# AdmiralenOla/Scoary

Hardware: AMD Instinct MI355X
Metric: gene x permutation Fisher tests/sec (higher is better)
Workload: dtype u32 bit-words (bit-sliced adders / AND + popcount), f64 for Fisher p; 1 GPU; cfg3: 50000 genes x 2000 isolates x 10 traits, --permute 10000 per GPU; counts + Fisher + label permutations + exceedance counts; gene_kind=config, gene_order=config, gene_partition=every rank its own genes (weak scaling), genes_per_gpu=50000, genes_total=50000, isolates=2000, traits=10, permutations=10000, parallelism=gene-shard x1, hip_graph=False, hip_graph_auto=False, label_tiles=generated on every rank, exchange=none (single GPU)

## Files before the change

include/scoary_hip.h:

```cpp
#ifndef SCOARY_HIP_H
#define SCOARY_HIP_H

#include <stdint.h>

#ifdef __cplusplus
extern "C" {
#endif

#define SCOARY_ABI_VERSION 11

#define SCOARY_OK 0
#define SCOARY_ERR_ARG (-1)
#define SCOARY_ERR_HIP (-2)
#define SCOARY_ERR_SIZE (-3)
#define SCOARY_ERR_DEVICE (-4)

typedef struct scoary_ctx *scoary_handle;
typedef void *scoary_stream_t;

int scoary_abi_version(void);

int scoary_create(int device, scoary_handle *out);
void scoary_destroy(scoary_handle h);
const char *scoary_last_error(scoary_handle h);
// ... 1 lines not shown
int64_t scoary_tiled_quads(int64_t N);
int64_t scoary_tiled_genes(int64_t G);
int64_t scoary_tiled_bytes(int64_t G, int64_t N);
int64_t scoary_row_words(int64_t N);

int scoary_pack_dense(scoary_handle h, const uint8_t *d_dense, int64_t G,
                      int64_t N, uint32_t *d_tiled, scoary_stream_t stream);
int scoary_tile_rows(scoary_handle h, const uint64_t *d_rows64, int64_t G,
                     int64_t N, uint32_t *d_tiled, scoary_stream_t stream);

int scoary_counts(scoary_handle h, const uint32_t *d_tiled,
                  const uint32_t *d_traits, const uint32_t *d_masks, int64_t G,
                  int64_t T, int64_t N, int32_t *d_counts, int32_t *d_margins,
                  scoary_stream_t stream);
int64_t scoary_counts_traits_per_pass(int64_t T);
int64_t scoary_trait_plan_bytes(int64_t T, int64_t N);
int scoary_trait_plan(scoary_handle h, const uint32_t *d_traits, const uint32_t *d_masks,
                      int64_t T, int64_t N, int32_t *d_margins, int32_t *d_mask_class,
                      void *d_plan, scoary_stream_t stream);
int scoary_counts_planned(scoary_handle h, const uint32_t *d_tiled, const void *d_plan,
                          const int32_t *d_margins, int64_t G, int64_t T, int64_t N,
                          int32_t *d_counts, scoary_stream_t stream);

int scoary_fisher(scoary_handle h, const int32_t *d_tables, int64_t M,
                  double *d_p, double *d_or, uint32_t *d_crit,
                  scoary_stream_t stream);
int64_t scoary_fisher_scipy_max_isolates(void);
int scoary_fisher_scipy(scoary_handle h, const int32_t *d_tables, int64_t M, double *d_p,
                        uint64_t *d_skipped, scoary_stream_t stream);
int scoary_fisher_lists(scoary_handle h, const int32_t *d_tables, int64_t T, int64_t G,
                        const int32_t *d_lorder, const uint8_t *d_lflipped,
                        double *d_p, double *d_or, uint32_t *d_crit, uint32_t *d_lcrit,
                        scoary_stream_t stream);

int64_t scoary_perm_max_isolates(void);
int scoary_perm_generate(scoary_handle h, const uint32_t *d_masks,
                         const int32_t *d_margins, int64_t T, int64_t N,
                         int64_t P, int64_t perm_base, int64_t trait_base,
                         uint64_t seed, uint32_t *d_perms, scoary_stream_t stream);

int scoary_permute(scoary_handle h, const uint32_t *d_tiled,
                   const uint32_t *d_perms, const uint32_t *d_crit, int64_t G,
                   int64_t T, int64_t N, int64_t P, uint32_t *d_r,
                   scoary_stream_t stream);

int scoary_permute_seq(scoary_handle h, const uint32_t *d_tiled, const uint32_t *d_perms,
                       const uint32_t *d_crit, const uint32_t *d_thr, int64_t G, int64_t T,
                       int64_t N, int64_t P, int64_t perm_base, uint32_t *d_r,
                       uint32_t *d_nstop, scoary_stream_t stream);

int64_t scoary_minp_fill_scratch_bytes(int64_t entries);
int scoary_minp_plan(scoary_handle h, const int32_t *d_counts, int64_t T, int64_t G, int64_t *d_off,
                     int32_t *d_lo, int64_t *entries_out, scoary_stream_t stream);
int scoary_minp_fill(scoary_handle h, const int32_t *d_counts, const int64_t *d_off,
                     const int32_t *d_lo, int64_t T, int64_t G, int64_t entries, void *d_scratch,
                     double *d_tab, scoary_stream_t stream);
int scoary_permute_minp(scoary_handle h, const uint32_t *d_tiled, const uint32_t *d_perms,
                        const int64_t *d_off, const int32_t *d_lo, const double *d_tab, int64_t G,
                        int64_t T, int64_t N, int64_t P, int64_t perm_base, int64_t minp_stride,
                        double *d_minp, scoary_stream_t stream);

int64_t scoary_stepdown_chunks(scoary_handle h, int64_t G, int64_t T, int64_t P);
int64_t scoary_stepdown_scratch_bytes(scoary_handle h, int64_t G, int64_t T, int64_t N, int64_t P);
int scoary_permute_stepdown(scoary_handle h, const uint32_t *d_tiled, const uint32_t *d_perms,
                            const int64_t *d_off, const int32_t *d_lo, const double *d_tab,
                            const int32_t *d_order, const double *d_psorted, int64_t G, int64_t T,
                            int64_t N, int64_t P, int64_t perm_base, int64_t minp_stride,
                            double *d_minp, uint32_t *d_c, void *d_scratch, scoary_stream_t stream);

int64_t scoary_list_tiles_words(int64_t N, int64_t P, int64_t T);
int64_t scoary_list_tile_words(int64_t N);
int64_t scoary_list_max_isolates(void);
int64_t scoary_list_segments(int64_t N);
int scoary_list_params(int64_t N, int64_t *out5);
int scoary_perm_generate_tiles(scoary_handle h, const uint32_t *d_masks,
                               const int32_t *d_margins, int64_t T, int64_t N, int64_t P,
                               int64_t perm_base, int64_t trait_base, uint64_t seed,
                               uint32_t *d_tiles, scoary_stream_t stream);
int scoary_perm_generate_tiles_range(scoary_handle h, const uint32_t *d_masks,
                                     const int32_t *d_margins, int64_t T, int64_t N, int64_t P,
                                     int64_t perm_base, int64_t trait_base, uint64_t seed,
                                     int64_t first_tile, int64_t n_tiles, uint32_t *d_tiles,
                                     scoary_stream_t stream);
int scoary_perm_max_strata(void);
int64_t scoary_perm_strata_max_isolates(void);
int scoary_strata_margins(scoary_handle h, const uint32_t *d_labels, const uint32_t *d_masks,
                          const uint16_t *d_strata, int64_t T, int64_t N, int64_t S,
                          int32_t *d_smargins, scoary_stream_t stream);
int scoary_perm_generate_strata(scoary_handle h, const uint32_t *d_masks, const uint16_t *d_strata,
                                const int32_t *d_members, const int32_t *d_offsets,
                                const int32_t *d_smargins, int64_t T, int64_t N, int64_t S, int64_t P,
                                int64_t perm_base, int64_t trait_base, uint64_t seed,
                                uint32_t *d_perms, scoary_stream_t stream);
int scoary_perm_generate_tiles_strata_range(scoary_handle h, const uint32_t *d_masks,
                                            const uint16_t *d_strata, const int32_t *d_members,
                                            const int32_t *d_offsets, const int32_t *d_smargins,
                                            int64_t T, int64_t N, int64_t S, int64_t P,
                                            int64_t perm_base, int64_t trait_base, uint64_t seed,
                                            int64_t first_tile, int64_t n_tiles, uint32_t *d_tiles,
                                            scoary_stream_t stream);
int64_t scoary_cmh_scratch_bytes(int64_t N);
int scoary_cmh(scoary_handle h, const uint32_t *d_tiled, const uint32_t *d_labels, const uint32_t *d_masks,
               const uint16_t *d_strata, const int32_t *d_members, const int32_t *d_offsets,
               const int32_t *d_smargins, int64_t G, int64_t T, int64_t N, int64_t S, double *d_stat,
               double *d_p, double *d_odds, double *d_e2, double *d_var, int32_t *d_a, uint32_t *d_crit,
               int32_t *d_scounts, void *d_scratch, scoary_stream_t stream);
int scoary_cmh_minp_plan(scoary_handle h, const uint32_t *d_tiled, const uint32_t *d_masks,
                         const uint16_t *d_strata, const int32_t *d_members, const int32_t *d_offsets,
                         const int32_t *d_smargins, int64_t G, int64_t T, int64_t N, int64_t S,
                         void *d_scratch, int64_t *d_off, int32_t *d_lo, int64_t *entries_out,
                         scoary_stream_t stream);
int scoary_cmh_minp_fill(scoary_handle h, const double *d_e2, const double *d_var, const int64_t *d_off,
                         const int32_t *d_lo, int64_t T, int64_t G, int64_t entries, double *d_tab,
                         scoary_stream_t stream);
int64_t scoary_cmh_exact_max_isolates(void);
int scoary_cmh_exact(scoary_handle h, const uint32_t *d_tiled, const uint32_t *d_masks, const uint16_t *d_strata,
                     const int32_t *d_members, const int32_t *d_offsets, const int32_t *d_smargins, int64_t G,
                     int64_t T, int64_t N, int64_t S, const int32_t *d_a, const uint32_t *d_crit,
                     const int64_t *d_off, const int32_t *d_lo, int64_t entries, double *d_p, double *d_p_region,
                     double *d_tab, void *d_scratch, scoary_stream_t stream);
int scoary_cmh_exact_odds(scoary_handle h, const uint32_t *d_tiled, const uint32_t *d_masks,
                          const uint16_t *d_strata, const int32_t *d_members, const int32_t *d_offsets,
                          const int32_t *d_smargins, int64_t G, int64_t T, int64_t N, int64_t S,
                          const int32_t *d_a, const int64_t *d_off, const int32_t *d_lo, int64_t entries, double half,
                          double *d_or, double *d_or_lo, double *d_or_hi, void *d_scratch,
                          scoary_stream_t stream);
int scoary_cmh_homogeneity(scoary_handle h, const uint32_t *d_tiled, const uint32_t *d_labels,
                           const uint32_t *d_masks, const uint16_t *d_strata, const int32_t *d_members,
                           const int32_t *d_offsets, const int32_t *d_smargins, int64_t G, int64_t T, int64_t N,
                           int64_t S, const double *d_odds, double *d_stat_bd, double *d_stat_tarone, int32_t *d_df,
                           double *d_p, void *d_scratch, scoary_stream_t stream);
int64_t scoary_permute_lists_scratch_bytes(int64_t G, int64_t T, int64_t N, int64_t P);
int scoary_permute_lists(scoary_handle h, const uint32_t *d_tiles, const uint32_t *d_lidx,
                         int64_t entries, const int32_t *d_lstart, const int32_t *d_lngroups,
                         const int32_t *d_lorder, const uint8_t *d_lflipped,
                         const uint32_t *d_crit, const uint32_t *d_lcrit,
                         const int32_t *d_margins, void *d_scratch,
                         int64_t G, int64_t T, int64_t N, int64_t P, uint32_t *d_r,
                         int accumulate, scoary_stream_t stream);

#define SCOARY_MFMA_ROUTE_NONE 0
#define SCOARY_MFMA_ROUTE_ALL 1
#define SCOARY_MFMA_ROUTE_AUTO 2
int64_t scoary_mfma_max_isolates(void);
int64_t scoary_mfma_panels_bytes(int64_t G, int64_t N);
int64_t scoary_mfma_bfrag_bytes(int64_t N, int64_t P, int64_t T);
int64_t scoary_mfma_breakeven_entries(void);
int scoary_mfma_panels_build(scoary_handle h, const uint32_t *d_tiled, int64_t G, int64_t N,
                             const int32_t *d_order, const uint8_t *d_flipped, void *d_panels,
                             scoary_stream_t stream);
int scoary_set_mfma_route(scoary_handle h, int mode);
int64_t scoary_mfma_route(scoary_handle h, const int64_t *block_start, int64_t G, int64_t T,
                          int64_t N, int64_t P);
int scoary_permute_hybrid(scoary_handle h, const uint32_t *d_tiles, const uint32_t *d_lidx,
                          int64_t entries, const int32_t *d_lstart, const int32_t *d_lngroups,
                          const int32_t *d_lorder, const uint8_t *d_lflipped,
                          const uint32_t *d_crit, const uint32_t *d_lcrit,
                          const int32_t *d_margins, void *d_scratch,
                          int64_t G, int64_t T, int64_t N, int64_t P, uint32_t *d_r,
                          int accumulate, const void *d_panels, void *d_bfrag, int64_t k_split,
                          int64_t routed_entries, scoary_stream_t stream);

int64_t scoary_lists_scratch_bytes(int64_t G, int64_t N);
int64_t scoary_lists_slack_entries(void);
int scoary_lists_plan(scoary_handle h, const uint32_t *d_tiled, int64_t G, int64_t N,
                      void *d_scratch, int32_t *d_start, int32_t *d_ngroups, int32_t *d_order,
                      uint8_t *d_flipped, int64_t *entries_out, scoary_stream_t stream);
int scoary_lists_fill(scoary_handle h, const uint32_t *d_tiled, int64_t G, int64_t N,
                      const void *d_scratch, const int32_t *d_order, const uint8_t *d_flipped,
                      int64_t entries, uint32_t *d_idx, scoary_stream_t stream);


int scoary_hamming(scoary_handle h, const uint32_t *d_tiled, const uint32_t *d_vecrows,
                   int64_t R, int64_t N, int32_t *d_out, scoary_stream_t stream);

int64_t scoary_upgma_scratch_bytes(int64_t n);
int scoary_upgma(scoary_handle h, const int32_t *d_counts, int64_t n, int64_t ncols, void *d_scratch,
                 int32_t *d_merges, int32_t *d_status, scoary_stream_t stream);

int scoary_gather_bits(scoary_handle h, const uint32_t *d_rows, int64_t R, int64_t Wsrc,
                       const int32_t *d_index, int64_t K, uint32_t *d_out,
                       scoary_stream_t stream);

int scoary_tree_pairs(scoary_handle h, const int32_t *d_ops, int64_t nops, int64_t stack_depth,
                      const uint32_t *d_gene_bits, const uint32_t *d_label_bits, int64_t G,
                      int64_t L, int64_t K, int32_t *d_out, scoary_stream_t stream);

int scoary_tree_permute(scoary_handle h, const int32_t *d_ops, int64_t nops,
                        int64_t stack_depth, const uint32_t *d_gene_bits,
                        const uint32_t *d_label_bits, int64_t G, int64_t L, int64_t K,
                        const int32_t *d_obs, uint8_t *d_exceed, scoary_stream_t stream);

int scoary_row_hash(scoary_handle h, const uint32_t *d_tiled, const uint32_t *d_masks,
                    int64_t G, int64_t T, int64_t N, uint64_t *d_out, scoary_stream_t stream);

int scoary_pack_records(scoary_handle h, const int32_t *d_counts, const double *d_p,
                        const double *d_odds, const uint32_t *d_r, const uint32_t *d_nstop,
                        int64_t M, uint32_t *d_rec, scoary_stream_t stream);

int scoary_gather(scoary_handle h, void *rccl_dl, void *comm, const void *d_send, void *d_recv,
                  int64_t bytes, int rank, int nranks, int root, scoary_stream_t stream);

typedef struct scoary_graph *scoary_graph_t;
int scoary_graph_begin(scoary_handle h, scoary_stream_t stream);
int scoary_graph_end(scoary_handle h, scoary_stream_t stream, scoary_graph_t *out);
int scoary_graph_launch(scoary_handle h, scoary_graph_t g, scoary_stream_t stream);
void scoary_graph_destroy(scoary_graph_t g);

int scoary_set_timing(scoary_handle h, int enabled);
int scoary_last_kernel_ms(scoary_handle h, const char *kernel, double *ms_out);

#ifdef __cplusplus
}
#endif
#endif
```

scoary_amd/_abi.py:

```python
import ctypes
import os

_HERE = os.path.dirname(os.path.abspath(__file__))
LIB_PATH = os.environ.get("SCOARY_HIP_LIB") or os.path.join(_HERE, "csrc", "libscoary_hip.so")
HEADER_PATH = os.path.join(os.path.dirname(_HERE), "include", "scoary_hip.h")

ABI_VERSION = 11
PERM_MAX_STRATA = 1024
PERM_STRATA_MAX_ISOLATES = 20479

_i64, _u64, _i32, _vp, _cp = (ctypes.c_int64, ctypes.c_uint64, ctypes.c_int,
                              ctypes.c_void_p, ctypes.c_char_p)

SIGNATURES = {
    "scoary_abi_version": (_i32, []),
    "scoary_create": (_i32, [_i32, ctypes.POINTER(_vp)]),
    "scoary_destroy": (None, [_vp]),
    "scoary_last_error": (_cp, [_vp]),
    "scoary_tiled_quads": (_i64, [_i64]),
    "scoary_tiled_genes": (_i64, [_i64]),
    "scoary_tiled_bytes": (_i64, [_i64, _i64]),
    "scoary_row_words": (_i64, [_i64]),
    "scoary_pack_dense": (_i32, [_vp, _vp, _i64, _i64, _vp, _vp]),
    "scoary_tile_rows": (_i32, [_vp, _vp, _i64, _i64, _vp, _vp]),
    "scoary_counts": (_i32, [_vp, _vp, _vp, _vp, _i64, _i64, _i64, _vp, _vp, _vp]),
    "scoary_counts_traits_per_pass": (_i64, [_i64]),
    "scoary_trait_plan_bytes": (_i64, [_i64, _i64]),
    "scoary_trait_plan": (_i32, [_vp, _vp, _vp, _i64, _i64, _vp, _vp, _vp, _vp]),
    "scoary_counts_planned": (_i32, [_vp, _vp, _vp, _vp, _i64, _i64, _i64, _vp, _vp]),
    "scoary_fisher": (_i32, [_vp, _vp, _i64, _vp, _vp, _vp, _vp]),
    "scoary_fisher_lists": (_i32, [_vp, _vp, _i64, _i64] + [_vp] * 7),
    "scoary_fisher_scipy": (_i32, [_vp, _vp, _i64, _vp, _vp, _vp]),
    "scoary_fisher_scipy_max_isolates": (_i64, []),
    "scoary_perm_generate": (_i32, [_vp, _vp, _vp, _i64, _i64, _i64, _i64, _i64, _u64, _vp, _vp]),
    "scoary_permute": (_i32, [_vp, _vp, _vp, _vp, _i64, _i64, _i64, _i64, _vp, _vp]),
    "scoary_permute_seq": (_i32, [_vp, _vp, _vp, _vp, _vp, _i64, _i64, _i64, _i64, _i64, _vp, _vp,
                                  _vp]),
    "scoary_minp_fill_scratch_bytes": (_i64, [_i64]),
    "scoary_minp_plan": (_i32, [_vp, _vp, _i64, _i64, _vp, _vp, ctypes.POINTER(_i64), _vp]),
    "scoary_minp_fill": (_i32, [_vp, _vp, _vp, _vp, _i64, _i64, _i64, _vp, _vp, _vp]),
    "scoary_permute_minp": (_i32, [_vp] * 6 + [_i64] * 6 + [_vp, _vp]),
    "scoary_stepdown_chunks": (_i64, [_vp, _i64, _i64, _i64]),
    "scoary_stepdown_scratch_bytes": (_i64, [_vp, _i64, _i64, _i64, _i64]),
    "scoary_permute_stepdown": (_i32, [_vp] * 8 + [_i64] * 6 + [_vp] * 4),
    "scoary_list_tiles_words": (_i64, [_i64, _i64, _i64]),
    "scoary_list_tile_words": (_i64, [_i64]),
    "scoary_list_params": (_i32, [_i64, _vp]),
    "scoary_list_max_isolates": (_i64, []),
    "scoary_list_segments": (_i64, [_i64]),
    "scoary_perm_generate_tiles": (_i32, [_vp, _vp, _vp, _i64, _i64, _i64, _i64, _i64, _u64, _vp,
                                          _vp]),
    "scoary_perm_generate_tiles_range": (_i32, [_vp, _vp, _vp, _i64, _i64, _i64, _i64, _i64, _u64, _i64,
                                                _i64, _vp, _vp]),
    "scoary_perm_max_isolates": (_i64, []),
    "scoary_perm_max_strata": (_i32, []),
    "scoary_perm_strata_max_isolates": (_i64, []),
    "scoary_strata_margins": (_i32, [_vp, _vp, _vp, _vp, _i64, _i64, _i64, _vp, _vp]),
    "scoary_perm_generate_strata": (_i32, [_vp] * 6 + [_i64] * 6 + [_u64, _vp, _vp]),
    "scoary_perm_generate_tiles_strata_range": (_i32, [_vp] * 6 + [_i64] * 6 + [_u64, _i64, _i64, _vp, _vp]),
    "scoary_cmh_scratch_bytes": (_i64, [_i64]),
    "scoary_cmh": (_i32, [_vp] * 8 + [_i64] * 4 + [_vp] * 10),
    "scoary_cmh_minp_plan": (_i32, [_vp] * 7 + [_i64] * 4 + [_vp] * 3 + [ctypes.POINTER(_i64), _vp]),
    "scoary_cmh_minp_fill": (_i32, [_vp] * 5 + [_i64] * 3 + [_vp, _vp]),
    "scoary_cmh_exact_max_isolates": (_i64, []),
    "scoary_cmh_exact": (_i32, [_vp] * 7 + [_i64] * 4 + [_vp] * 4 + [_i64] + [_vp] * 5),
    "scoary_cmh_exact_odds": (_i32, [_vp] * 7 + [_i64] * 4 + [_vp] * 3 + [_i64, ctypes.c_double] + [_vp] * 5),
    "scoary_cmh_homogeneity": (_i32, [_vp] * 8 + [_i64] * 4 + [_vp] * 7),
    "scoary_permute_lists_scratch_bytes": (_i64, [_i64, _i64, _i64, _i64]),
    "scoary_permute_lists": (_i32, [_vp, _vp, _vp, _i64] + [_vp] * 8 + [_i64, _i64, _i64, _i64, _vp,
                                                                       _i32, _vp]),
    "scoary_mfma_max_isolates": (_i64, []),
    "scoary_mfma_panels_bytes": (_i64, [_i64, _i64]),
    "scoary_mfma_bfrag_bytes": (_i64, [_i64, _i64, _i64]),
    "scoary_mfma_breakeven_entries": (_i64, []),
    "scoary_mfma_panels_build": (_i32, [_vp, _vp, _i64, _i64, _vp, _vp, _vp, _vp]),
    "scoary_set_mfma_route": (_i32, [_vp, _i32]),
    "scoary_mfma_route": (_i64, [_vp, _vp, _i64, _i64, _i64, _i64]),
    "scoary_permute_hybrid": (_i32, [_vp, _vp, _vp, _i64] + [_vp] * 8 + [_i64, _i64, _i64, _i64, _vp,
                                                                        _i32, _vp, _vp, _i64, _i64, _vp]),
    "scoary_lists_scratch_bytes": (_i64, [_i64, _i64]),
    "scoary_lists_slack_entries": (_i64, []),
    "scoary_lists_plan": (_i32, [_vp, _vp, _i64, _i64, _vp, _vp, _vp, _vp, _vp,
                                 ctypes.POINTER(_i64), _vp]),
    "scoary_lists_fill": (_i32, [_vp, _vp, _i64, _i64, _vp, _vp, _vp, _i64, _vp, _vp]),
    "scoary_hamming": (_i32, [_vp, _vp, _vp, _i64, _i64, _vp, _vp]),
    "scoary_upgma_scratch_bytes": (_i64, [_i64]),
    "scoary_upgma": (_i32, [_vp, _vp, _i64, _i64, _vp, _vp, _vp, _vp]),
    "scoary_gather_bits": (_i32, [_vp, _vp, _i64, _i64, _vp, _i64, _vp, _vp]),
    "scoary_tree_pairs": (_i32, [_vp, _vp, _i64, _i64, _vp, _vp, _i64, _i64, _i64, _vp, _vp]),
    "scoary_tree_permute": (_i32, [_vp, _vp, _i64, _i64, _vp, _vp, _i64, _i64, _i64, _vp, _vp,
                                   _vp]),
    "scoary_row_hash": (_i32, [_vp, _vp, _vp, _i64, _i64, _i64, _vp, _vp]),
    "scoary_pack_records": (_i32, [_vp, _vp, _vp, _vp, _vp, _vp, _i64, _vp, _vp]),
    "scoary_gather": (_i32, [_vp, _vp, _vp, _vp, _vp, _i64, _i32, _i32, _i32, _vp]),
    "scoary_graph_begin": (_i32, [_vp, _vp]),
    "scoary_graph_end": (_i32, [_vp, _vp, ctypes.POINTER(_vp)]),
    "scoary_graph_launch": (_i32, [_vp, _vp, _vp]),
    "scoary_graph_destroy": (None, [_vp]),
    "scoary_set_timing": (_i32, [_vp, _i32]),
    "scoary_last_kernel_ms": (_i32, [_vp, _cp, ctypes.POINTER(ctypes.c_double)]),
}

_lib = None


class ScoaryHipError(RuntimeError):
    pass


def load():
    global _lib
    if _lib is not None:
        return _lib
    if not os.path.exists(LIB_PATH):
        raise ScoaryHipError(
            "HIP extension not built: %s is missing. Run "
            "`python -c 'import __graft_entry__ as g; g.build()'` (needs hipcc). "
            "scoary_amd has no CPU fallback." % LIB_PATH)
    try:
        import torch
    except ImportError:
        pass
    lib = ctypes.CDLL(LIB_PATH, mode=ctypes.RTLD_GLOBAL)
    for name, (res, args) in SIGNATURES.items():
        fn = getattr(lib, name)
        fn.restype = res
        fn.argtypes = args
    got = lib.scoary_abi_version()
    if got != ABI_VERSION:
        raise ScoaryHipError("ABI version mismatch: library %d, binding %d" % (got, ABI_VERSION))
    if (lib.scoary_perm_max_strata(), lib.scoary_perm_strata_max_isolates()) != \
            (PERM_MAX_STRATA, PERM_STRATA_MAX_ISOLATES):
        raise ScoaryHipError("the library's strata limits differ from the binding's")
    _lib = lib
    return lib
```

scoary_amd/csrc/scoary_common.hpp:

```cpp
#ifndef SCOARY_COMMON_HPP
#define SCOARY_COMMON_HPP
#include <hip/hip_runtime.h>

#include <algorithm>
#include <cmath>
#include <cstdint>
#include <cstdio>
#include <cstdlib>
#include <cstring>
#include <string>
#include <utility>
#include <vector>

#include "scoary_hip.h"

struct scoary_ctx {
  int device = 0;
  int num_cu = 256;
  std::string err;
  bool timing = false;
  int lists_lds_optin = 0;
  int labels_lds_optin = 0;
  int mfma_lds_optin = 0;
  int cmh_exact_lds_optin = 0;
  int cmh_exact_odds_lds_optin = 0;
  int mfma_route = SCOARY_MFMA_ROUTE_AUTO;
  uint32_t* scipy_primes = nullptr;
  float* scipy_inv = nullptr;
  int scipy_nprimes = 0;
  struct Timed {
    std::string name;
    hipEvent_t start, stop;
  };
  std::vector<Timed> timed;
};

struct MfmaGeom {
  int64_t stages, rp, per, gene_blocks, blocks;
};
MfmaGeom scoary_mfma_geom(int num_cu, int64_t k_split, int64_t T, int64_t P, int64_t ntiles);
int scoary_mfma_launch(scoary_handle h, hipStream_t s, const uint32_t* d_tiles, const void* d_panels, void* d_bfrag,
                       const uint32_t* d_lcrit, uint16_t* d_partial, int64_t k_split, int64_t G, int64_t T,
                       int64_t N, int64_t P, int64_t ntiles, int64_t gs);

int scoary_cmh_segments_launch(scoary_handle h, hipStream_t s, const uint16_t* d_strata, const int32_t* d_members,
                               int64_t N, int64_t S, void* d_scratch, const char* event);

namespace {

constexpr int kWave = 64;
constexpr int kGeneAlign = 256;

using RegQuads = std::integer_sequence<int, 1, 2, 4, 6, 8, 12, 16, 20, 24>;
constexpr int kChunkQuads = 8;

template <int... Q>
constexpr int quads_at_least(std::integer_sequence<int, Q...>, int64_t q) {
  int r = 0;
  ((r = (Q >= q && (r == 0 || Q < r)) ? Q : r), ...);
  return r;
}
template <int... Q>
constexpr int quads_max(std::integer_sequence<int, Q...>) {
  int r = 0;
  ((r = Q > r ? Q : r), ...);
  return r;
}
constexpr int kMaxRegQuads = quads_max(RegQuads{});

template <int... Q, class F>
inline bool with_quads(std::integer_sequence<int, Q...>, int64_t Qp, F&& f) {
  return ((Qp == Q && (f(std::integral_constant<int, Q>{}), true)) || ...);
}
template <class F>
inline bool with_reg_quads(int64_t Qp, F&& f) {
  return with_quads(RegQuads{}, Qp, f);
}

inline int64_t round_up(int64_t x, int64_t m) { return (x + m - 1) / m * m; }

inline int64_t tiled_quads(int64_t N) {
  int64_t q = (((N + 31) / 32) + 3) / 4;
  if (q < 1) q = 1;
  const int r = quads_at_least(RegQuads{}, q);
  return r ? r : round_up(q, kChunkQuads);
}

inline bool tiled_quads_ok(int64_t Qp) {
  return Qp > kMaxRegQuads ? Qp % kChunkQuads == 0 : with_reg_quads(Qp, [](auto) {});
}

constexpr int kSegRows = 20352;
constexpr int kSegTW = 2;
constexpr int kSegStride = ((kSegRows + 1) * kSegTW + 3) / 4 * 4;
constexpr int kSegPiece = 8;
constexpr int kMaxListIsolates = 131070;
__host__ __device__ constexpr int list_segments(int64_t N) {
  return N <= 20479 ? 1 : (N <= kMaxListIsolates ? (int)((N + kSegRows - 1) / kSegRows) : 0);
}
__host__ __device__ constexpr int list_tw(int64_t N) {
  return N <= 2559 ? 16 : (N <= 5119 ? 8 : (N <= 10239 ? 4 : (list_segments(N) ? 2 : 0)));
}
__host__ __device__ constexpr int list_lpg(int TW) { return TW >= 4 ? TW / 4 : 1; }
__host__ __device__ constexpr int list_nw(int TW) { return TW >= 4 ? 4 : TW; }
__host__ __device__ constexpr int64_t list_tile_dwords(int64_t N, int TW) {
  return ((N + 1) * TW + 3) / 4 * 4;
}
__host__ __device__ constexpr int64_t list_tile_dwords_seg(int64_t N, int TW) {
  return list_segments(N) > 1 ? (int64_t)list_segments(N) * kSegStride : list_tile_dwords(N, TW);
}
__host__ __device__ constexpr int64_t list_seg_rows(int64_t N, int s) {
  return list_segments(N) > 1 ? (N - (int64_t)s * kSegRows < kSegRows ? N - (int64_t)s * kSegRows : kSegRows) : N;
}
__host__ __device__ constexpr int64_t list_row_dword(int64_t N, int64_t row) {
  return list_segments(N) > 1 ? row / kSegRows * kSegStride + row % kSegRows * kSegTW : row * kSegTW;
}

constexpr int kListPad = 16;
constexpr int kListStartUnit = 32;
constexpr int kListChunkMB = 2;
constexpr int kListSlack = 256;

int fail(scoary_handle h, int code, const std::string& msg) {
  if (h) h->err = msg;
  return code;
}

inline int check_args(scoary_handle h, const char* what, bool ok) {
  return ok ? SCOARY_OK : fail(h, SCOARY_ERR_ARG, std::string(what) + ": bad argument");
}
inline int strata_check(scoary_handle h, const char* what, bool ok, int64_t T, int64_t N, int64_t S) {
  if (int rc = check_args(h, what, ok && T >= 1 && N >= 1 && S >= 1)) return rc;
  if (T > 65535) return fail(h, SCOARY_ERR_SIZE, std::string(what) + ": T > 65535");
  if (S > scoary_perm_max_strata())
    return fail(h, SCOARY_ERR_SIZE, std::string(what) + ": more strata than scoary_perm_max_strata()");
  if (N > scoary_perm_strata_max_isolates())
    return fail(h, SCOARY_ERR_SIZE, std::string(what) + ": more isolates than scoary_perm_strata_max_isolates()");
  return SCOARY_OK;
}

#define HIP_TRY(h, expr)                                                              \
  do {                                                                                \
    hipError_t e_ = (expr);                                                           \
    if (e_ != hipSuccess)                                                             \
      return fail(h, SCOARY_ERR_HIP, std::string(#expr) + ": " + hipGetErrorString(e_)); \
  } while (0)

struct DeviceGuard {
  int prev = -1;
  bool switched = false;
  explicit DeviceGuard(int dev) {
    if (hipGetDevice(&prev) == hipSuccess && prev != dev) switched = (hipSetDevice(dev) == hipSuccess);
  }
  ~DeviceGuard() {
    if (switched) (void)hipSetDevice(prev);
  }
};

struct KernelTimer {
  scoary_handle h;
  hipStream_t s;
  hipEvent_t start = nullptr, stop = nullptr;
  KernelTimer(scoary_handle h_, hipStream_t s_, const char* name) : h(h_), s(s_) {
    if (!name || !h->timing) return;
    if (hipEventCreate(&start) != hipSuccess || hipEventCreate(&stop) != hipSuccess) {
      start = stop = nullptr;
      return;
    }
    (void)hipEventRecord(start, s);
    h->timed.push_back({name, start, stop});
  }
  ~KernelTimer() {
    if (stop) (void)hipEventRecord(stop, s);
  }
};

__device__ __forceinline__ void philox4x32_10(uint32_t c0, uint32_t c1, uint32_t c2, uint32_t c3,
                                              uint32_t k0, uint32_t k1, uint32_t (&out)[4]) {
#pragma unroll
  for (int r = 0; r < 10; ++r) {
    const uint64_t p0 = (uint64_t)0xD2511F53u * c0, p1 = (uint64_t)0xCD9E8D57u * c2;
    const uint32_t h0 = (uint32_t)(p0 >> 32), l0 = (uint32_t)p0;
    const uint32_t h1 = (uint32_t)(p1 >> 32), l1 = (uint32_t)p1;
    const uint32_t n0 = __builtin_amdgcn_bitop3_b32(h1, c1, k0, 0x96), n2 = __builtin_amdgcn_bitop3_b32(h0, c3, k1, 0x96);
    c0 = n0;
    c1 = l1;
    c2 = n2;
    c3 = l0;
    k0 += 0x9E3779B9u;
    k1 += 0xBB67AE85u;
  }
// ... 64 lines not shown
```

scoary_amd/csrc/scoary_mfma.hip:

```cpp
#include "scoary_common.hpp"

const double kMfmaNsPerGene = 62.0;
const double kListNsPerEntry = 0.177;
const double kMfmaPanelLoadStages = 10.0;

namespace {

typedef int v8i __attribute__((ext_vector_type(8)));
typedef int v4i __attribute__((ext_vector_type(4)));
typedef float v16f __attribute__((ext_vector_type(16)));

constexpr int kKSteps = 32;
constexpr int kBlockGenes = 256;
constexpr int kBlockWaves = 8;
constexpr int kFragBytes = 1024;
constexpr int kStageBytes = 2 * kKSteps * kFragBytes;
constexpr int kHalfBytes = kStageBytes / 2;
constexpr int kRingSlots = 4;
constexpr int kAhead = kRingSlots - 2;
constexpr int kRingBytes = kRingSlots * kHalfBytes;
constexpr int kDmaPerHalf = kHalfBytes / kBlockWaves / kFragBytes;
constexpr int kMfmaLds = kRingBytes;
static_assert(kRingSlots >= 4 && kMfmaLds <= 160 * 1024 && (kAhead - 1) * kDmaPerHalf < 64,
              "a half stage is issued at least two ticks ahead, within the LDS of a CU and the vmcnt field");

__device__ __forceinline__ uint32_t fp4_of_bits8(uint32_t b) {
  uint32_t y = b | (b << 12);
  y = (y | (y << 6)) & 0x03030303u;
  return __builtin_amdgcn_perm(0u, 0x22200200u, y);
}
__device__ __forceinline__ v4i fp4_of_bits32(uint32_t w) {
  return v4i{(int)fp4_of_bits8(w & 0xffu), (int)fp4_of_bits8((w >> 8) & 0xffu),
             (int)fp4_of_bits8((w >> 16) & 0xffu), (int)fp4_of_bits8(w >> 24)};
}

__global__ __launch_bounds__(256) void k_mfma_panels(const uint32_t* __restrict__ tiled, int64_t Gp, int G, int N,
                                                     const int32_t* __restrict__ order,
                                                     const uint8_t* __restrict__ flipped, int64_t total,
                                                     v4i* __restrict__ panels) {
  const int64_t idx = (int64_t)blockIdx.x * 256 + threadIdx.x;
  if (idx >= total) return;
  const int lane = (int)(idx & 63);
  const int64_t f = idx >> 6;
  const int k = (int)(f & 31), i = (int)((f >> 5) & 1);
  const int64_t slot = (f >> 6) * 64 + i * 32 + (lane & 31);
  const int w = 2 * k + (lane >> 5);
  uint32_t bits = 0u;
  if (slot < G && 32 * w < N) {
    const int g = order[slot];
    bits = tiled[((int64_t)(w >> 2) * Gp + g) * 4 + (w & 3)];
    if (flipped[g]) bits = ~bits;
    if (32 * w + 32 > N) bits &= (1u << (N - 32 * w)) - 1u;
  }
  panels[idx] = fp4_of_bits32(bits);
}

__global__ __launch_bounds__(256) void k_mfma_bfrag(const uint32_t* __restrict__ tiles, int N, int ntiles,
                                                    int64_t tile_dwords, int S, v4i* __restrict__ bfrag) {
  const int s = blockIdx.x, t = blockIdx.y;
  const int lane = threadIdx.x & 63, wave = threadIdx.x >> 6;
  const uint32_t* tile = tiles + ((int64_t)t * ntiles + (s >> 3)) * tile_dwords + 2 * (s & 7);
  v4i* out = bfrag + ((int64_t)t * S + s) * (kStageBytes / 16);
  for (int k = wave; k < kKSteps; k += 4) {
    const int row = k * 64 + lane;
    uint2 w = make_uint2(0u, 0u);
    if (row < N) w = *reinterpret_cast<const uint2*>(tile + (int64_t)row * 16);
#pragma unroll
    for (int j = 0; j < 2; ++j) {
      const uint32_t x = j ? w.y : w.x;
      uint32_t mine = 0u;
#pragma unroll
      for (int c = 0; c < 32; ++c) {
        const uint64_t bal = __ballot((x >> c) & 1u);
        const uint32_t v = (lane >> 5) ? (uint32_t)(bal >> 32) : (uint32_t)bal;
        if ((lane & 31) == c) mine = v;
      }
      out[(k * 2 + j) * 64 + lane] = fp4_of_bits32(mine);
    }
  }
}

__device__ __forceinline__ void mfma_dma16(uint32_t lds, uint32_t lane_off, const unsigned char* src) {
  uint32_t m0_saved;
  asm volatile("s_mov_b32 %0, m0\n\ts_mov_b32 m0, %1\n\ts_nop 0\n\t"
               "global_load_lds_dwordx4 %2, %3\n\ts_mov_b32 m0, %0"
               : "=&s"(m0_saved)
               : "s"(lds), "v"(lane_off), "s"(src)
               : "memory");
}

__device__ __forceinline__ int xcd_item(int orig, int n) {
  const int q = n >> 3, r = n & 7, x = orig & 7;
  return (x < r ? x * (q + 1) : r * (q + 1) + (x - r) * q) + (orig >> 3);
}

__global__ __launch_bounds__(kBlockWaves * 64) __attribute__((amdgpu_waves_per_eu(2, 2)))
void k_permute_mfma(const v4i* __restrict__ panels, const unsigned char* __restrict__ bfrag,
                    const uint2* __restrict__ lcrit, int G, int64_t P, int S, int per, int rp, int nblk_genes,
                    int ntiles, int64_t gs, uint16_t* __restrict__ partial) {
  extern __shared__ __attribute__((aligned(16))) unsigned char lds[];
  const int item = xcd_item(blockIdx.x, gridDim.x);
  const int gb = item % nblk_genes, rng = item / nblk_genes;
  const int t = rng / rp, jr = rng % rp;
  const int s0 = jr * per, ns = min(per, S - s0);
  const int tid = threadIdx.x, lane = tid & 63, half = lane >> 5, l31 = lane & 31;
  const int wave = __builtin_amdgcn_readfirstlane(tid >> 6);
  const bool late = wave >= kBlockWaves / 2;
  const int64_t row0 = (int64_t)gb * kBlockGenes + wave * 32 + 4 * half;
  v16f negc;
  float hw[16];
#pragma unroll
  for (int r = 0; r < 16; ++r) {
    const int64_t slot = row0 + (r & 3) + 8 * (r >> 2);
    const uint2 cr = lcrit[(int64_t)t * G + min(slot, (int64_t)G - 1)];
    negc[r] = -0.5f * (float)((int)cr.x + (int)cr.y - 1);
    hw[r] = slot < G ? 0.5f * (float)((int)cr.y - 1 - (int)cr.x) : 1e30f;
  }
  v4i a[kKSteps];
  {
    const v4i* ap = panels + ((int64_t)gb * kBlockWaves + wave) * (kKSteps * 64) + lane;
#pragma unroll
    for (int k = 0; k < kKSteps; ++k) a[k] = ap[k * 64];
#pragma unroll
    for (int k = 0; k < kKSteps; ++k) asm volatile("" : "+v"(a[k]));
    asm volatile("" : "+v"(negc));
#pragma unroll
    for (int r = 0; r < 16; ++r) asm volatile("" : "+v"(hw[r]));
  }

  const uint32_t lds0 = (uint32_t)(uintptr_t)(const __attribute__((address_space(3))) unsigned char*)lds;
  const uint32_t lane_off = (uint32_t)lane * 16u;
  const unsigned char* bsrc = bfrag + ((int64_t)t * S + s0) * kStageBytes + wave * (kHalfBytes / kBlockWaves);
  const int nh = 2 * ns;
  auto issue_half = [&](int n) {
    const unsigned char* src = bsrc + (int64_t)min(n, nh - 1) * kHalfBytes;
    const uint32_t dst = lds0 + (uint32_t)(n % kRingSlots) * kHalfBytes + (uint32_t)wave * (kHalfBytes / kBlockWaves);
#pragma unroll
    for (int p = 0; p < kDmaPerHalf; ++p) mfma_dma16(dst + p * kFragBytes, lane_off, src + p * kFragBytes);
  };
#pragma unroll
  for (int n = 0; n < kAhead; ++n) issue_half(n);
  int tick = 0;
  auto next_tick = [&]() {
    asm volatile("s_waitcnt vmcnt(%0)" ::"n"((kAhead - 1) * kDmaPerHalf) : "memory");
    __builtin_amdgcn_s_barrier();
    issue_half(tick + kAhead);
    ++tick;
  };

  uint32_t ex[16];
#pragma unroll
  for (int r = 0; r < 16; ++r) ex[r] = 0u;
  const int64_t last_valid = P - (int64_t)s0 * 64;

  v16f acc[2];
  auto region_test = [&](int64_t nvalid) {
    if (nvalid >= 64) {
#pragma unroll
      for (int r = 0; r < 16; ++r)
        ex[r] += (uint32_t)(__builtin_fabsf(acc[0][r]) > hw[r]) + (uint32_t)(__builtin_fabsf(acc[1][r]) > hw[r]);
    } else {
      const bool v0 = l31 < nvalid, v1 = l31 + 32 < nvalid;
#pragma unroll
      for (int r = 0; r < 16; ++r)
        ex[r] += (uint32_t)(v0 && __builtin_fabsf(acc[0][r]) > hw[r]) +
                 (uint32_t)(v1 && __builtin_fabsf(acc[1][r]) > hw[r]);
    }
  };
  if (late) next_tick();
  int rslot = 0;
  for (int st = 0; st < ns; ++st) {
#pragma unroll
    for (int h = 0; h < 2; ++h) {
      next_tick();
      const unsigned char* bbuf = lds + rslot * kHalfBytes + lane * 16;
      rslot = rslot == kRingSlots - 1 ? 0 : rslot + 1;
      v4i bq[3][2];
      auto read_b = [&](int kk) {
#pragma unroll
        for (int j = 0; j < 2; ++j)
          bq[kk % 3][j] = *reinterpret_cast<const v4i*>(bbuf + (kk * 2 + j) * kFragBytes);
      };
      read_b(0);
      read_b(1);
      if (h == 0) {
        __builtin_amdgcn_sched_barrier(0);
        if (st > 0) region_test(64);
        __builtin_amdgcn_sched_barrier(0);
      }
#pragma unroll
      for (int kk = 0; kk < kKSteps / 2; ++kk) {
        const int k = h * (kKSteps / 2) + kk;
        if (kk + 2 < kKSteps / 2) read_b(kk + 2);
        __builtin_amdgcn_sched_barrier(0);
        const v8i aa = v8i{a[k].x, a[k].y, a[k].z, a[k].w, 0, 0, 0, 0};
#pragma unroll
        for (int j = 0; j < 2; ++j) {
          const v4i x = bq[kk % 3][j];
          acc[j] = __builtin_amdgcn_mfma_scale_f32_32x32x64_f8f6f4(aa, v8i{x.x, x.y, x.z, x.w, 0, 0, 0, 0},
                                                                   k == 0 ? negc : acc[j], 4, 4, 0, 0x7f7f7f7f, 0,
                                                                   0x7f7f7f7f);
        }
        __builtin_amdgcn_sched_barrier(0);
      }
    }
  }
  if (!late) next_tick();
  region_test(last_valid - (int64_t)(ns - 1) * 64);
  asm volatile("s_waitcnt vmcnt(0)" ::: "memory");

  uint16_t* out = partial + ((int64_t)t * ntiles + jr) * gs + row0;
  const int nrows = (int)min((int64_t)32, (int64_t)G - ((int64_t)gb * kBlockGenes + wave * 32));
#pragma unroll
  for (int r = 0; r < 16; ++r) {
    uint32_t v = ex[r];
#pragma unroll
    for (int off = 16; off > 0; off >>= 1) v += __shfl_xor(v, off);
    const int row = (r & 3) + 8 * (r >> 2);
    if (l31 == 0 && 4 * half + row < nrows) {
      out[row] = (uint16_t)v;
      for (int tile = jr + rp; tile < ntiles; tile += rp) out[(int64_t)(tile - jr) * gs + row] = 0;
    }
  }
}

}

MfmaGeom scoary_mfma_geom(int num_cu, int64_t k_split, int64_t T, int64_t P, int64_t ntiles) {
  MfmaGeom g{};
  g.stages = (P + 63) / 64;
  g.gene_blocks = (k_split + kBlockGenes - 1) / kBlockGenes;
  const int64_t rp_min = (g.stages + 1022) / 1023, rp_max = std::min<int64_t>(std::min(ntiles, g.stages), 64);
  double best = 0.0;
  for (int64_t rp = rp_min; rp <= std::max(rp_min, rp_max); ++rp) {
    const int64_t per = (g.stages + rp - 1) / rp, ranges = (g.stages + per - 1) / per;
    const int64_t blocks = g.gene_blocks * T * ranges;
    const double cost = (double)((blocks + num_cu - 1) / num_cu) * ((double)per + kMfmaPanelLoadStages);
    if (g.rp == 0 || cost < best) best = cost, g.rp = ranges, g.per = per, g.blocks = blocks;
  }
  return g;
}

int scoary_mfma_launch(scoary_handle h, hipStream_t s, const uint32_t* d_tiles, const void* d_panels, void* d_bfrag,
                       const uint32_t* d_lcrit, uint16_t* d_partial, int64_t k_split, int64_t G, int64_t T,
                       int64_t N, int64_t P, int64_t ntiles, int64_t gs) {
  const MfmaGeom g = scoary_mfma_geom(h->num_cu, k_split, T, P, ntiles);
  if (g.blocks > 0x7fffffffLL || g.stages > 0x7fffffffLL / 64)
    return fail(h, SCOARY_ERR_SIZE, "scoary_permute_hybrid: grid too large");
  if (!h->mfma_lds_optin) {
    HIP_TRY(h, hipFuncSetAttribute(reinterpret_cast<const void*>(&k_permute_mfma),
                                   hipFuncAttributeMaxDynamicSharedMemorySize, 160 * 1024));
    h->mfma_lds_optin = 1;
  }
  {
    KernelTimer kt(h, s, "k_mfma_bfrag");
    hipLaunchKernelGGL(k_mfma_bfrag, dim3((unsigned)g.stages, (unsigned)T), dim3(256), 0, s, d_tiles, (int)N,
                       (int)ntiles, list_tile_dwords(N, 16), (int)g.stages, static_cast<v4i*>(d_bfrag));
  }
  {
    KernelTimer kt(h, s, "k_permute_mfma");
    hipLaunchKernelGGL(k_permute_mfma, dim3((unsigned)g.blocks), dim3(kBlockWaves * 64), kMfmaLds, s,
                       static_cast<const v4i*>(d_panels), static_cast<const unsigned char*>(d_bfrag),
                       reinterpret_cast<const uint2*>(d_lcrit), (int)G, P, (int)g.stages, (int)g.per, (int)g.rp,
                       (int)g.gene_blocks, (int)ntiles, gs, d_partial);
  }
  HIP_TRY(h, hipGetLastError());
  return SCOARY_OK;
}

extern "C" {

int64_t scoary_mfma_max_isolates(void) { return kKSteps * 64; }
int64_t scoary_mfma_panels_bytes(int64_t G, int64_t N) {
  if (G < 1 || N < 1 || N > kKSteps * 64) return 0;
  return round_up(G, kBlockGenes) * (2 * kKSteps * 16);
}
int64_t scoary_mfma_bfrag_bytes(int64_t N, int64_t P, int64_t T) {
  if (N < 1 || N > kKSteps * 64 || P < 1 || T < 1) return 0;
  return T * ((P + 63) / 64) * kStageBytes;
}
int64_t scoary_mfma_breakeven_entries(void) { return (int64_t)std::ceil(kMfmaNsPerGene / kListNsPerEntry); }

int scoary_mfma_panels_build(scoary_handle h, const uint32_t* d_tiled, int64_t G, int64_t N, const int32_t* d_order,
                             const uint8_t* d_flipped, void* d_panels, scoary_stream_t stream) {
  if (!h) return SCOARY_ERR_ARG;
  if (!d_tiled || !d_order || !d_flipped || !d_panels || G < 1 || N < 1)
    return fail(h, SCOARY_ERR_ARG, "scoary_mfma_panels_build: bad argument");
  if (N > kKSteps * 64 || G > 0x7fffffffLL - kBlockGenes)
    return fail(h, SCOARY_ERR_SIZE, "scoary_mfma_panels_build: N > 2048 or G >= 2^31");
  DeviceGuard guard(h->device);
  hipStream_t s = static_cast<hipStream_t>(stream);
  const int64_t total = scoary_mfma_panels_bytes(G, N) / 16;
  KernelTimer kt(h, s, "k_mfma_panels");
  hipLaunchKernelGGL(k_mfma_panels, dim3((unsigned)((total + 255) / 256)), dim3(256), 0, s, d_tiled,
                     scoary_tiled_genes(G), (int)G, (int)N, d_order, d_flipped, total, static_cast<v4i*>(d_panels));
  HIP_TRY(h, hipGetLastError());
  return SCOARY_OK;
}

int scoary_set_mfma_route(scoary_handle h, int mode) {
  if (!h) return SCOARY_ERR_ARG;
  if (mode < SCOARY_MFMA_ROUTE_NONE || mode > SCOARY_MFMA_ROUTE_AUTO)
    return fail(h, SCOARY_ERR_ARG, "scoary_set_mfma_route: mode is 0 (none), 1 (all) or 2 (auto)");
  h->mfma_route = mode;
  return SCOARY_OK;
}

int64_t scoary_mfma_route(scoary_handle h, const int64_t* block_start, int64_t G, int64_t T, int64_t N, int64_t P) {
  if (!h || G < 1 || T < 1 || P < 1 || N < 1 || N > kKSteps * 64 || h->mfma_route == SCOARY_MFMA_ROUTE_NONE)
    return 0;
  if (h->mfma_route == SCOARY_MFMA_ROUTE_ALL) return G;
  if (!block_start) return 0;
  const int64_t nb = G / kBlockGenes, total = block_start[(G + kBlockGenes - 1) / kBlockGenes];
  const double tests = (double)T * (double)P / 1e5;
  const double stage_ns = kMfmaNsPerGene * h->num_cu * kBlockGenes * 64 / 1e5;
  double best = kListNsPerEntry * (double)total * tests;
  int64_t best_nb = 0;
  for (int64_t b = 1; b <= nb; ++b) {
    const MfmaGeom g = scoary_mfma_geom(h->num_cu, b * kBlockGenes, T, P, (P + 511) / 512);
    if (g.blocks < h->num_cu) continue;
    const double cost = (double)((g.blocks + h->num_cu - 1) / h->num_cu) * ((double)g.per + kMfmaPanelLoadStages) * stage_ns +
                        kListNsPerEntry * (double)(total - block_start[b]) * tests;
    if (cost < best) best = cost, best_nb = b;
  }
  return best_nb * kBlockGenes;
}

}
```

Baseline: 1893 billion tests/s.

## Let MFMA permutation blocks span trait boundaries with flattened trait-stage ranges

Work ranges for the MFMA permutation kernel now cover a flattened (trait, stage) index space instead of per-trait stage ranges, so a block can cross trait boundaries. Per-trait thresholds are prefetched into LDS with DMA before the switch, and partial counts are flushed at each segment end. A new cost model that includes block-start and trait-switch terms picks the range length, with the aim of better load balance across CUs and fewer fixed per-block panel loads. The change adds kernel complexity and more LDS per block, and it alters the routing heuristic constants.

```diff
diff --git a/include/scoary_hip.h b/include/scoary_hip.h
--- a/include/scoary_hip.h
+++ b/include/scoary_hip.h
@@ -177,6 +177,7 @@
 int scoary_set_mfma_route(scoary_handle h, int mode);
 int64_t scoary_mfma_route(scoary_handle h, const int64_t *block_start, int64_t G, int64_t T,
                           int64_t N, int64_t P);
+int scoary_mfma_plan(int num_cu, int64_t k_split, int64_t T, int64_t P, int64_t *out);
 int scoary_permute_hybrid(scoary_handle h, const uint32_t *d_tiles, const uint32_t *d_lidx,
                           int64_t entries, const int32_t *d_lstart, const int32_t *d_lngroups,
                           const int32_t *d_lorder, const uint8_t *d_lflipped,
diff --git a/scoary_amd/_abi.py b/scoary_amd/_abi.py
--- a/scoary_amd/_abi.py
+++ b/scoary_amd/_abi.py
@@ -76,6 +76,7 @@
     "scoary_mfma_panels_build": (_i32, [_vp, _vp, _i64, _i64, _vp, _vp, _vp, _vp]),
     "scoary_set_mfma_route": (_i32, [_vp, _i32]),
     "scoary_mfma_route": (_i64, [_vp, _vp, _i64, _i64, _i64, _i64]),
+    "scoary_mfma_plan": (_i32, [_i32, _i64, _i64, _i64, ctypes.POINTER(_i64)]),
     "scoary_permute_hybrid": (_i32, [_vp, _vp, _vp, _i64] + [_vp] * 8 + [_i64, _i64, _i64, _i64, _vp,
                                                                         _i32, _vp, _vp, _i64, _i64, _vp]),
     "scoary_lists_scratch_bytes": (_i64, [_i64, _i64]),
diff --git a/scoary_amd/csrc/scoary_common.hpp b/scoary_amd/csrc/scoary_common.hpp
--- a/scoary_amd/csrc/scoary_common.hpp
+++ b/scoary_amd/csrc/scoary_common.hpp
@@ -36,7 +36,8 @@
 };
 
 struct MfmaGeom {
-  int64_t stages, rp, per, gene_blocks, blocks;
+  int64_t stages, Q, ranges, L, gene_blocks, blocks;
+  double cost;
 };
 MfmaGeom scoary_mfma_geom(int num_cu, int64_t k_split, int64_t T, int64_t P, int64_t ntiles);
 int scoary_mfma_launch(scoary_handle h, hipStream_t s, const uint32_t* d_tiles, const void* d_panels, void* d_bfrag,
diff --git a/scoary_amd/csrc/scoary_mfma.hip b/scoary_amd/csrc/scoary_mfma.hip
--- a/scoary_amd/csrc/scoary_mfma.hip
+++ b/scoary_amd/csrc/scoary_mfma.hip
@@ -1,8 +1,9 @@
 #include "scoary_common.hpp"
 
-const double kMfmaNsPerGene = 62.0;
-const double kListNsPerEntry = 0.177;
-const double kMfmaPanelLoadStages = 10.0;
+const double kMfmaNsPerGene = 58.0;
+const double kListNsPerEntry = 0.18;
+const double kMfmaBlockStartStages = 6.0;
+const double kMfmaTraitSwitchStages = 2.0;
 
 namespace {
 
@@ -20,7 +21,8 @@
 constexpr int kAhead = kRingSlots - 2;
 constexpr int kRingBytes = kRingSlots * kHalfBytes;
 constexpr int kDmaPerHalf = kHalfBytes / kBlockWaves / kFragBytes;
-constexpr int kMfmaLds = kRingBytes;
+constexpr int kThrBytes = 32 * 8;
+constexpr int kMfmaLds = kRingBytes + kBlockWaves * kThrBytes;
 static_assert(kRingSlots >= 4 && kMfmaLds <= 160 * 1024 && (kAhead - 1) * kDmaPerHalf < 64,
               "a half stage is issued at least two ticks ahead, within the LDS of a CU and the vmcnt field");
 
@@ -89,6 +91,15 @@
                : "memory");
 }
 
+__device__ __forceinline__ void mfma_dma4(uint32_t lds, uint32_t lane_off, const unsigned char* src) {
+  uint32_t m0_saved;
+  asm volatile("s_mov_b32 %0, m0\n\ts_mov_b32 m0, %1\n\ts_nop 0\n\t"
+               "global_load_lds_dword %2, %3\n\ts_mov_b32 m0, %0"
+               : "=&s"(m0_saved)
+               : "s"(lds), "v"(lane_off), "s"(src)
+               : "memory");
+}
+
 __device__ __forceinline__ int xcd_item(int orig, int n) {
   const int q = n >> 3, r = n & 7, x = orig & 7;
   return (x < r ? x * (q + 1) : r * (q + 1) + (x - r) * q) + (orig >> 3);
@@ -96,41 +107,61 @@
 
 __global__ __launch_bounds__(kBlockWaves * 64) __attribute__((amdgpu_waves_per_eu(2, 2)))
 void k_permute_mfma(const v4i* __restrict__ panels, const unsigned char* __restrict__ bfrag,
-                    const uint2* __restrict__ lcrit, int G, int64_t P, int S, int per, int rp, int nblk_genes,
+                    const uint2* __restrict__ lcrit, int G, int64_t P, int S, int64_t Q, int L, int nblk_genes,
                     int ntiles, int64_t gs, uint16_t* __restrict__ partial) {
   extern __shared__ __attribute__((aligned(16))) unsigned char lds[];
   const int item = xcd_item(blockIdx.x, gridDim.x);
   const int gb = item % nblk_genes, rng = item / nblk_genes;
-  const int t = rng / rp, jr = rng % rp;
-  const int s0 = jr * per, ns = min(per, S - s0);
+  const int64_t q0 = (int64_t)rng * L;
+  const int ns = (int)min((int64_t)L, Q - q0);
+  int t = (int)(q0 / S), s = (int)(q0 % S);
+  int jt = rng - (int)((int64_t)t * S / L);
   const int tid = threadIdx.x, lane = tid & 63, half = lane >> 5, l31 = lane & 31;
   const int wave = __builtin_amdgcn_readfirstlane(tid >> 6);
   const bool late = wave >= kBlockWaves / 2;
-  const int64_t row0 = (int64_t)gb * kBlockGenes + wave * 32 + 4 * half;
+  const int wslot0 = gb * kBlockGenes + wave * 32;
+  const int rows_mine = min(32, G - wslot0) - 4 * half;
   v16f negc;
   float hw[16];
-#pragma unroll
-  for (int r = 0; r < 16; ++r) {
-    const int64_t slot = row0 + (r & 3) + 8 * (r >> 2);
-    const uint2 cr = lcrit[(int64_t)t * G + min(slot, (int64_t)G - 1)];
-    negc[r] = -0.5f * (float)((int)cr.x + (int)cr.y - 1);
-    hw[r] = slot < G ? 0.5f * (float)((int)cr.y - 1 - (int)cr.x) : 1e30f;
-  }
+  const uint32_t lds0 = (uint32_t)(uintptr_t)(const __attribute__((address_space(3))) unsigned char*)lds;
+  const uint32_t lane_off = (uint32_t)lane * 16u;
+  const int thr_slot0 = min(wslot0, G - 1);
+  const uint32_t thr_lds = kRingBytes + (uint32_t)wave * kThrBytes;
+  auto fetch_thresholds = [&](int tt) {
+    uint32_t l = lane_off;
+    asm volatile("" : "+v"(l));
+    l >>= 4;
+    const uint32_t off = (uint32_t)min((int)(l >> 1), G - 1 - thr_slot0) * 8u + (l & 1u) * 4u;
+    mfma_dma4(lds0 + thr_lds, off, reinterpret_cast<const unsigned char*>(lcrit + ((int64_t)tt * G + thr_slot0)));
+  };
+  auto take_thresholds = [&]() {
+    int h4 = 4 * half, mine = rows_mine;
+    asm volatile("" : "+v"(h4), "+v"(mine));
+    const uint2* thr = reinterpret_cast<const uint2*>(lds + thr_lds) + h4;
+#pragma unroll
+    for (int r = 0; r < 16; ++r) {
+      const int row = (r & 3) + 8 * (r >> 2);
+      const uint2 cr = thr[row];
+      negc[r] = -0.5f * (float)((int)cr.x + (int)cr.y - 1);
+      hw[r] = row < mine ? 0.5f * (float)((int)cr.y - 1 - (int)cr.x) : 1e30f;
+    }
+    asm volatile("" : "+v"(negc));
+#pragma unroll
+    for (int r = 0; r < 16; ++r) asm volatile("" : "+v"(hw[r]));
+  };
   v4i a[kKSteps];
   {
+    fetch_thresholds(t);
     const v4i* ap = panels + ((int64_t)gb * kBlockWaves + wave) * (kKSteps * 64) + lane;
 #pragma unroll
     for (int k = 0; k < kKSteps; ++k) a[k] = ap[k * 64];
 #pragma unroll
     for (int k = 0; k < kKSteps; ++k) asm volatile("" : "+v"(a[k]));
-    asm volatile("" : "+v"(negc));
-#pragma unroll
-    for (int r = 0; r < 16; ++r) asm volatile("" : "+v"(hw[r]));
-  }
-
-  const uint32_t lds0 = (uint32_t)(uintptr_t)(const __attribute__((address_space(3))) unsigned char*)lds;
-  const uint32_t lane_off = (uint32_t)lane * 16u;
-  const unsigned char* bsrc = bfrag + ((int64_t)t * S + s0) * kStageBytes + wave * (kHalfBytes / kBlockWaves);
+    asm volatile("s_waitcnt vmcnt(0)" ::: "memory");
+    take_thresholds();
+  }
+
+  const unsigned char* bsrc = bfrag + q0 * kStageBytes + wave * (kHalfBytes / kBlockWaves);
   const int nh = 2 * ns;
   auto issue_half = [&](int n) {
     const unsigned char* src = bsrc + (int64_t)min(n, nh - 1) * kHalfBytes;
@@ -151,21 +182,39 @@
   uint32_t ex[16];
 #pragma unroll
   for (int r = 0; r < 16; ++r) ex[r] = 0u;
-  const int64_t last_valid = P - (int64_t)s0 * 64;
+  const int ragged = (int)(P - (int64_t)(S - 1) * 64);
 
   v16f acc[2];
-  auto region_test = [&](int64_t nvalid) {
-    if (nvalid >= 64) {
-#pragma unroll
-      for (int r = 0; r < 16; ++r)
-        ex[r] += (uint32_t)(__builtin_fabsf(acc[0][r]) > hw[r]) + (uint32_t)(__builtin_fabsf(acc[1][r]) > hw[r]);
-    } else {
+  auto region_test = [&](int nvalid) {
+    if (nvalid < 64) {
       const bool v0 = l31 < nvalid, v1 = l31 + 32 < nvalid;
 #pragma unroll
-      for (int r = 0; r < 16; ++r)
-        ex[r] += (uint32_t)(v0 && __builtin_fabsf(acc[0][r]) > hw[r]) +
-                 (uint32_t)(v1 && __builtin_fabsf(acc[1][r]) > hw[r]);
-    }
+      for (int r = 0; r < 16; ++r) {
+        acc[0][r] = v0 ? acc[0][r] : __builtin_nanf("");
+        acc[1][r] = v1 ? acc[1][r] : __builtin_nanf("");
+      }
+    }
+#pragma unroll
+    for (int r = 0; r < 16; ++r)
+      ex[r] += (uint32_t)(__builtin_fabsf(acc[0][r]) > hw[r]) + (uint32_t)(__builtin_fabsf(acc[1][r]) > hw[r]);
+  };
+  const int jt0 = jt;
+  auto end_segment = [&](int tt) {
+    uint16_t* out = partial + ((int64_t)tt * ntiles + jt) * gs + wslot0;
+    int rl = l31, h4 = 4 * half, mine = rows_mine;
+    asm volatile("" : "+v"(rl), "+v"(h4), "+v"(mine));
+    uint32_t count = 0u;
+#pragma unroll
+    for (int r = 0; r < 16; ++r) {
+      uint32_t v = ex[r];
+#pragma unroll
+      for (int off = 16; off > 0; off >>= 1) v += __shfl_xor(v, off);
+      ex[r] = 0u;
+      count = rl == r ? v : count;
+    }
+    const int row = (rl & 3) + 8 * (rl >> 2);
+    if (rl < 16 && row < mine) out[h4 + row] = (uint16_t)count;
+    jt = 0;
   };
   if (late) next_tick();
   int rslot = 0;
@@ -185,7 +234,15 @@
       read_b(1);
       if (h == 0) {
         __builtin_amdgcn_sched_barrier(0);
-        if (st > 0) region_test(64);
+        if (st > 0) {
+          const bool entered = s == 0;
+          region_test(entered ? ragged : 64);
+          if (entered) {
+            end_segment(t - 1);
+            take_thresholds();
+          }
+        }
+        if (s == S - 1 && st + 1 < ns) fetch_thresholds(t + 1);
         __builtin_amdgcn_sched_barrier(0);
       }
 #pragma unroll
@@ -204,41 +261,67 @@
         __builtin_amdgcn_sched_barrier(0);
       }
     }
+    if (++s == S) s = 0, ++t;
   }
   if (!late) next_tick();
-  region_test(last_valid - (int64_t)(ns - 1) * 64);
+  const bool trait_done = s == 0;
+  region_test(trait_done ? ragged : 64);
   asm volatile("s_waitcnt vmcnt(0)" ::: "memory");
-
-  uint16_t* out = partial + ((int64_t)t * ntiles + jr) * gs + row0;
-  const int nrows = (int)min((int64_t)32, (int64_t)G - ((int64_t)gb * kBlockGenes + wave * 32));
-#pragma unroll
-  for (int r = 0; r < 16; ++r) {
-    uint32_t v = ex[r];
-#pragma unroll
-    for (int off = 16; off > 0; off >>= 1) v += __shfl_xor(v, off);
-    const int row = (r & 3) + 8 * (r >> 2);
-    if (l31 == 0 && 4 * half + row < nrows) {
-      out[row] = (uint16_t)v;
-      for (int tile = jr + rp; tile < ntiles; tile += rp) out[(int64_t)(tile - jr) * gs + row] = 0;
-    }
-  }
-}
-
+  end_segment(trait_done ? t - 1 : t);
+
+  {
+    int rl = l31, h4 = 4 * half, mine = rows_mine;
+    asm volatile("" : "+v"(rl), "+v"(h4), "+v"(mine));
+    const int row = (rl & 3) + 8 * (rl >> 2);
+    const bool stores = rl < 16 && row < mine;
+    const int t0 = (int)(q0 / S);
+    for (int tt = t0; tt < t; ++tt) {
+      uint16_t* out = partial + (int64_t)tt * ntiles * gs + wslot0 + h4 + row;
+      for (int tile = (tt == t0 ? jt0 : 0) + 1; tile < ntiles; ++tile)
+        if (stores) out[(int64_t)tile * gs] = 0;
+    }
+  }
+}
+
+}
+
+struct MfmaRange {
+  int64_t L, ranges, switches;
+};
+static std::vector<MfmaRange> mfma_ranges(int64_t T, int64_t P, int64_t ntiles) {
+  std::vector<MfmaRange> out;
+  const int64_t S = (P + 63) / 64, Q = T * S;
+  for (int64_t L = std::min<int64_t>(Q, 1023); L >= 1; --L) {
+    const int64_t ranges = (Q + L - 1) / L;
+    if ((Q + ranges - 1) / ranges != L) continue;
+    bool ok = true;
+    for (int64_t t = 0; t < std::min(T, L) && ok; ++t) ok = ((t + 1) * S - 1) / L - t * S / L + 1 <= ntiles;
+    if (!ok) continue;
+    MfmaRange c{L, ranges, 0};
+    for (int64_t r = 0; r < std::min(ranges, S); ++r)
+      c.switches = std::max(c.switches, (std::min(Q, (r + 1) * L) - 1) / S - r * L / S);
+    out.push_back(c);
+  }
+  return out;
+}
+
+static MfmaGeom mfma_pick(const std::vector<MfmaRange>& cands, int num_cu, int64_t gene_blocks, int64_t S,
+                          int64_t T) {
+  MfmaGeom g{};
+  g.stages = S;
+  g.Q = T * S;
+  g.gene_blocks = gene_blocks;
+  for (const MfmaRange& c : cands) {
+    const int64_t blocks = gene_blocks * c.ranges;
+    const double cost = (double)((blocks + num_cu - 1) / num_cu) *
+                        ((double)c.L + kMfmaBlockStartStages + (double)c.switches * kMfmaTraitSwitchStages);
+    if (g.L == 0 || cost < g.cost) g.cost = cost, g.ranges = c.ranges, g.L = c.L, g.blocks = blocks;
+  }
+  return g;
 }
 
 MfmaGeom scoary_mfma_geom(int num_cu, int64_t k_split, int64_t T, int64_t P, int64_t ntiles) {
-  MfmaGeom g{};
-  g.stages = (P + 63) / 64;
-  g.gene_blocks = (k_split + kBlockGenes - 1) / kBlockGenes;
-  const int64_t rp_min = (g.stages + 1022) / 1023, rp_max = std::min<int64_t>(std::min(ntiles, g.stages), 64);
-  double best = 0.0;
-  for (int64_t rp = rp_min; rp <= std::max(rp_min, rp_max); ++rp) {
-    const int64_t per = (g.stages + rp - 1) / rp, ranges = (g.stages + per - 1) / per;
-    const int64_t blocks = g.gene_blocks * T * ranges;
-    const double cost = (double)((blocks + num_cu - 1) / num_cu) * ((double)per + kMfmaPanelLoadStages);
-    if (g.rp == 0 || cost < best) best = cost, g.rp = ranges, g.per = per, g.blocks = blocks;
-  }
-  return g;
+  return mfma_pick(mfma_ranges(T, P, ntiles), num_cu, (k_split + kBlockGenes - 1) / kBlockGenes, (P + 63) / 64, T);
 }
 
 int scoary_mfma_launch(scoary_handle h, hipStream_t s, const uint32_t* d_tiles, const void* d_panels, void* d_bfrag,
@@ -261,7 +344,7 @@
     KernelTimer kt(h, s, "k_permute_mfma");
     hipLaunchKernelGGL(k_permute_mfma, dim3((unsigned)g.blocks), dim3(kBlockWaves * 64), kMfmaLds, s,
                        static_cast<const v4i*>(d_panels), static_cast<const unsigned char*>(d_bfrag),
-                       reinterpret_cast<const uint2*>(d_lcrit), (int)G, P, (int)g.stages, (int)g.per, (int)g.rp,
+                       reinterpret_cast<const uint2*>(d_lcrit), (int)G, P, (int)g.stages, g.Q, (int)g.L,
                        (int)g.gene_blocks, (int)ntiles, gs, d_partial);
   }
   HIP_TRY(h, hipGetLastError());
@@ -298,6 +381,13 @@
   return SCOARY_OK;
 }
 
+int scoary_mfma_plan(int num_cu, int64_t k_split, int64_t T, int64_t P, int64_t* out) {
+  if (num_cu < 1 || k_split < 1 || T < 1 || P < 1 || !out) return SCOARY_ERR_ARG;
+  const MfmaGeom g = scoary_mfma_geom(num_cu, k_split, T, P, (P + 511) / 512);
+  out[0] = g.gene_blocks, out[1] = g.ranges, out[2] = g.L, out[3] = g.blocks;
+  return SCOARY_OK;
+}
+
 int scoary_set_mfma_route(scoary_handle h, int mode) {
   if (!h) return SCOARY_ERR_ARG;
   if (mode < SCOARY_MFMA_ROUTE_NONE || mode > SCOARY_MFMA_ROUTE_AUTO)
@@ -316,11 +406,11 @@
   const double stage_ns = kMfmaNsPerGene * h->num_cu * kBlockGenes * 64 / 1e5;
   double best = kListNsPerEntry * (double)total * tests;
   int64_t best_nb = 0;
+  const std::vector<MfmaRange> cands = mfma_ranges(T, P, (P + 511) / 512);
   for (int64_t b = 1; b <= nb; ++b) {
-    const MfmaGeom g = scoary_mfma_geom(h->num_cu, b * kBlockGenes, T, P, (P + 511) / 512);
+    const MfmaGeom g = mfma_pick(cands, h->num_cu, b, (P + 63) / 64, T);
     if (g.blocks < h->num_cu) continue;
-    const double cost = (double)((g.blocks + h->num_cu - 1) / h->num_cu) * ((double)g.per + kMfmaPanelLoadStages) * stage_ns +
-                        kListNsPerEntry * (double)(total - block_start[b]) * tests;
+    const double cost = g.cost * stage_ns + kListNsPerEntry * (double)(total - block_start[b]) * tests;
     if (cost < best) best = cost, best_nb = b;
   }
   return best_nb * kBlockGenes;
```

Measured after the change: 1957 billion tests/s, median of 6. +3.4%, better.
